# xinntao/EDVR

Hardware: AMD Instinct MI355X
Metric: EDVR-L x4 5-frame 720p clips/sec (higher is better)
Workload: dtype fp32 emulated as 2xf16 (hi+lo, 22-bit operands, 4 cross products), fp32 accumulate; 1 GPU; EDVR-L x4, 5 frames, 180x320 LR -> 720x1280, batch 10/GPU, inference; clips_per_gpu=10, global_clips=10, parallelism=clip-sharded x1, no data-path collective, world_size=1, backend=single process

## Files before the change

edvr_amd/_lib.py:

```python
import ctypes
import os

_HERE = os.path.dirname(os.path.abspath(__file__))
LIB_PATH = os.environ.get('EDVR_AMD_LIB') or os.path.join(_HERE, 'lib', 'libedvr_amd.so')

c_float_p = ctypes.c_void_p
i32, i64, f32, sz = ctypes.c_int, ctypes.c_int64, ctypes.c_float, ctypes.c_size_t
vp = ctypes.c_void_p


class ConvDesc(ctypes.Structure):
    _fields_ = [
        ('x1', vp), ('x2', vp), ('c1', i32), ('c2', i32), ('x1_img_stride', i64), ('x2_img_stride', i64),
        ('x2_div', i32), ('x2_mul', i32), ('x2_add', i32), ('n', i32), ('h', i32), ('w', i32), ('wpk', vp),
        ('bias', vp), ('co', i32), ('ks', i32), ('stride', i32), ('act', i32), ('act_from', i32), ('res1', vp),
        ('res2', vp), ('res1_img_stride', i64), ('res2_img_stride', i64), ('y', vp), ('y_img_stride', i64),
        ('out_mode', i32), ('algo', i32), ('gate', vp), ('gate_img_stride', i64), ('gate_slope', f32), ('y_scale', f32),
        ('wpk_f4', vp), ('abs_sum', vp), ('abs_sum_channels', i32), ('wpk_f4s', vp), ('x_amax', vp), ('y_amax', vp),
        ('pre', vp), ('pre_img_stride', i64), ('pre_div', i32), ('pre_mul', i32), ('pre_add', i32), ('pre_n', i32), ('wpk_ds', vp),
    ]


PROTOTYPES = {
    'edvr_version': (ctypes.c_char_p, []),
    'edvr_last_error': (ctypes.c_char_p, []),
    'edvr_check_device': (i32, []),
    'edvr_conv2d_packed_weight_elems': (sz, [i32, i32, i32]),
    'edvr_conv2d_pack_weight_f32': (i32, [vp, vp, i32, i32, i32, i32, vp]),
    'edvr_conv2d_packed_weight_f4_elems': (sz, [i32, i32]),
    'edvr_conv2d_pack_weight_f4_f32': (i32, [vp, vp, i32, i32, i32, vp]),
    'edvr_conv2d_packed_weight_f4s_elems': (sz, [i32, i32]),
    'edvr_conv2d_pack_weight_f4s_f32': (i32, [vp, vp, i32, i32, i32, vp]),
    'edvr_conv2d_packed_weight_1x1s_elems': (sz, [i32, i32]),
    'edvr_conv2d_pack_weight_1x1s_f32': (i32, [vp, vp, i32, i32, vp]),
    'edvr_conv2d_packed_weight_ds_elems': (sz, [i32, i32, i32]),
    'edvr_conv2d_pack_weight_ds_f32': (i32, [vp, vp, i32, i32, i32, vp]),
    'edvr_amax_f32': (i32, [vp, vp, i32, i64, i64, vp]),
    'edvr_pack_job_bytes': (sz, []),
    'edvr_conv2d_pack_weights_multi': (i32, [vp, i32, i32, i32, vp]),
    'edvr_conv2d_f32': (i32, [ctypes.POINTER(ConvDesc), vp]),
    'edvr_conv2d_kernel': (i32, [ctypes.POINTER(ConvDesc)]),
    'edvr_conv2d_gate_supported': (i32, [ctypes.POINTER(ConvDesc)]),
    'edvr_conv2d_abs_sum_supported': (i32, [ctypes.POINTER(ConvDesc)]),
    'edvr_conv2d_y_amax_supported': (i32, [ctypes.POINTER(ConvDesc)]),
    'edvr_conv2d_pre_supported': (i32, [ctypes.POINTER(ConvDesc)]),
    'edvr_conv2d_f4s_set_lean': (i32, [i32]),
    'edvr_conv2d_f4s_lean_items': (i32, [ctypes.POINTER(ConvDesc)]),
    'edvr_conv2d_kernel_name': (i32, [ctypes.POINTER(ConvDesc), ctypes.c_char_p, sz]),
    'edvr_conv2d_executed_flops': (i32, [ctypes.POINTER(ConvDesc), ctypes.POINTER(ctypes.c_double)]),
    'edvr_dcnv2_fwd_ws_bytes': (sz, [i32] * 12),
    'edvr_dcnv2_fwd_f32': (i32, [vp] * 6 + [i32] * 12 + [i64, i64, i32, i32, vp, sz, vp]),
    'edvr_dcnv2_fwd_split_f32': (i32, [vp] * 6 + [i32] * 12 + [i64, i64, i32, i32, vp, sz, vp, vp]),
    'edvr_dcnv2_fwd_split_applies': (i32, [vp] + [i32] * 13),
    'edvr_dcnv2_fwd_kernel_name': (i32, [vp] + [i32] * 13 + [ctypes.c_char_p, sz]),
    'edvr_dcnv2_bwd_ws_bytes': (sz, [i32] * 12),
    'edvr_dcnv2_any_ws_bytes': (sz, [i32] * 13),
    'edvr_dcnv2_fwd_any': (i32, [i32] + [vp] * 6 + [i32] * 12 + [i64, i64, vp, sz, vp]),
    'edvr_dcnv2_bwd_any': (i32, [i32] + [vp] * 10 + [i32] * 12 + [i64, i64, i64, i64, vp, sz, vp]),
    'edvr_psnr_sse_f32': (i32, [vp, vp, vp, i32, i32, i32, i32, i64, i64, i32, i32, i32, vp]),
    'edvr_ssim_partials': (sz, [i32, i32, i32]),
    'edvr_ssim_f32': (i32, [vp, vp, vp, i32, i32, i32, i32, i64, i64, i32, i32, vp]),
    'edvr_niqe_blocks': (sz, [i32, i32, i32]),
    'edvr_niqe_moments_f32': (i32, [vp, vp, i32, i32, i32, i32, i64, i32, vp]),
    'edvr_niqe_moments_u8': (i32, [vp, vp, i32, i32, i32, i64, i32, vp]),
    'edvr_frames_u8_to_f32': (i32, [vp, vp, i32, i32, i32, i32, vp, i32, vp]),
    'edvr_gather_images_f32': (i32, [vp, vp, vp, vp, i32, vp, i32, i32, vp]),
    'edvr_upsample4x_add_u8': (i32, [vp, vp, vp, i32, i32, i32, vp]),
    'edvr_f32_to_u8_hwc': (i32, [vp, vp, i32, i32, i32, i64, vp]),
    'edvr_crop_pad_frames_u8': (i32, [vp, vp, i32, i32, i32, i32, i32, i32, i32, i32, vp]),
# ... 98 lines not shown
```

edvr_amd/csrc/winograd_f4s.hip:

```cpp
#include <atomic>
#include <cstdlib>
#include <type_traits>

#include "common.h"
#include "pack.h"

#ifndef F4S_PLAIN
#define F4S_PLAIN 1
#endif

namespace edvr {

typedef float f32x16 __attribute__((ext_vector_type(16)));
typedef float f32x4 __attribute__((ext_vector_type(4)));
typedef float f32x2 __attribute__((ext_vector_type(2)));
typedef int i32x4 __attribute__((ext_vector_type(4)));
typedef _Float16 f16x8 __attribute__((ext_vector_type(8)));

__device__ __forceinline__ float max_raw_s(float a, float b) {
  float o;
  asm("v_max_f32 %0, %1, %2" : "=v"(o) : "v"(a), "v"(b));
  return o;
}

__device__ __forceinline__ void split6_f16x2(const float (&x)[6], float s, unsigned (&o)[6]) {
  asm volatile(
      "v_fma_mixlo_f16 %0, %6, %12, 0\n\tv_fma_mixlo_f16 %1, %7, %12, 0\n\tv_fma_mixlo_f16 %2, %8, %12, 0\n\t"
      "v_fma_mixlo_f16 %3, %9, %12, 0\n\tv_fma_mixlo_f16 %4, %10, %12, 0\n\tv_fma_mixlo_f16 %5, %11, %12, 0\n\t"
      "v_fma_mixhi_f16 %0, %6, %12, -%0 op_sel_hi:[0,0,1]\n\tv_fma_mixhi_f16 %1, %7, %12, -%1 op_sel_hi:[0,0,1]\n\t"
      "v_fma_mixhi_f16 %2, %8, %12, -%2 op_sel_hi:[0,0,1]\n\tv_fma_mixhi_f16 %3, %9, %12, -%3 op_sel_hi:[0,0,1]\n\t"
      "v_fma_mixhi_f16 %4, %10, %12, -%4 op_sel_hi:[0,0,1]\n\tv_fma_mixhi_f16 %5, %11, %12, -%5 op_sel_hi:[0,0,1]"
      : "=&v"(o[0]), "=&v"(o[1]), "=&v"(o[2]), "=&v"(o[3]), "=&v"(o[4]), "=&v"(o[5])
      : "v"(x[0]), "v"(x[1]), "v"(x[2]), "v"(x[3]), "v"(x[4]), "v"(x[5]), "s"(s));
}

struct WinoF4SArgs {
  edvr_conv2d_desc d;
  const unsigned *U;
  int ci, ci_real, cop, tiles_x, tiles_y, items;
  float ys, ys_gs;
  int lean;
};

#define F4S_LDS_BARRIER() asm volatile("s_waitcnt lgkmcnt(0)\n\ts_barrier" ::: "memory")

#ifdef F4S_PROF
__device__ unsigned long long f4s_prof[16 * 8];
#define F4S_NOW(v) asm volatile("s_memtime %0\n\ts_waitcnt lgkmcnt(0)" : "=s"(v)::"memory")
#define F4S_BARRIER_AT(slot)                                        \
  do {                                                              \
    unsigned long long a_, b_;                                      \
    asm volatile("s_waitcnt lgkmcnt(0)" ::: "memory");              \
    F4S_NOW(a_);                                                    \
    asm volatile("s_barrier" ::: "memory");                         \
    F4S_NOW(b_);                                                    \
    f4s_pc[slot] += (unsigned)(b_ - a_);                            \
  } while (0)
#define F4S_SPAN_BEGIN() F4S_NOW(f4s_t0)
#define F4S_SPAN_END(slot)                                          \
  do {                                                              \
    unsigned long long b_;                                          \
    F4S_NOW(b_);                                                    \
    f4s_pc[slot] += (unsigned)(b_ - f4s_t0);                        \
    f4s_t0 = b_;                                                    \
  } while (0)
#define F4S_WAIT_DMA()                                              \
  do {                                                              \
    unsigned long long a_, b_;                                      \
    F4S_NOW(a_);                                                    \
    asm volatile("s_waitcnt vmcnt(0)" ::: "memory");                \
    F4S_NOW(b_);                                                    \
    f4s_pc[4] += (unsigned)(b_ - a_);                               \
  } while (0)
#define F4S_PROF_FLUSH()                                                                                         \
  do {                                                                                                          \
    if ((threadIdx.x & 63) == 0)                                                                                \
      for (int i_ = 0; i_ < 8; ++i_) atomicAdd(&f4s_prof[(threadIdx.x >> 6) * 8 + i_], (unsigned long long)f4s_pc[i_]); \
  } while (0)
#else
#define F4S_BARRIER_AT(slot) F4S_LDS_BARRIER()
#define F4S_SPAN_BEGIN()
#define F4S_SPAN_END(slot)
#define F4S_WAIT_DMA() asm volatile("s_waitcnt vmcnt(0)" ::: "memory")
#define F4S_PROF_FLUSH()
#endif
#if defined(F4S_PROF) && F4S_PROF >= 2
#define F4S_POS_T0() unsigned long long pa_, pb_, pc_; F4S_NOW(pa_)
#define F4S_POS_T1()                                                \
  do {                                                              \
    F4S_NOW(pb_);                                                   \
    asm volatile("s_waitcnt vmcnt(5)" ::: "memory");                \
    F4S_NOW(pc_);                                                   \
    f4s_pc[5] += (unsigned)(pb_ - pa_);                             \
    f4s_pc[6] += (unsigned)(pc_ - pb_);                             \
  } while (0)
#else
#define F4S_POS_T0()
#define F4S_POS_T1()
#endif
#define F4S_BARRIER() F4S_BARRIER_AT(7)

__device__ __forceinline__ float f4s_input_scale(float amax) {
  const int be = (int)((__builtin_bit_cast(unsigned, amax) >> 23) & 255u);
  const int field = min(max(127 + 8 - (be - 127), 7), 227);
  return __builtin_bit_cast(float, (unsigned)field << 23);
}

template <int TXL>
__global__ __launch_bounds__(1024, 1) void conv3x3_winograd_f4s_kernel(const WinoF4SArgs a) {
  constexpr int TX = 1 << TXL, TY = 32 / TX;
  constexpr int BW = 4 * TX, BH = 4 * TY;
  constexpr int RROWS = BH + 2, RPIECES = TX + 2;
  static_assert(RROWS * RPIECES == 180, "a wave's region holds 2 x 180 pieces either way");
  constexpr int CK = 8;
  constexpr int VSLAB = CK * 36 * 32;
  constexpr int XSZ = 2 * 6 * 8 * 32 * 4;
  constexpr int RWAVE = 6 * 64 * 4 + 4;
  constexpr int UCHUNK = 6 * 2 * 6 * 1024;
  __shared__ __attribute__((aligned(16))) float smem[2 * VSLAB + XSZ + 4 * RWAVE + 64];
  float *const Xs = smem + 2 * VSLAB;
  float *const bias_s = smem + 2 * VSLAB + XSZ + 4 * RWAVE;

  const edvr_conv2d_desc &d = a.d;
  const int tid = threadIdx.x, lane = tid & 63, half = lane >> 5, j = lane & 31;
  const int wave = __builtin_amdgcn_readfirstlane(tid >> 6);
  const int hw = d.h * d.w, plane_bytes = hw * 4;
  const int co_blocks = (d.co + 63) / 64;
  const int n_chunks = a.ci / CK;
  constexpr int RSRC_FLAGS = 0x00020000;
  auto uniform_rsrc = [&](const void *p, int bytes) {
    const uint64_t pv = reinterpret_cast<uint64_t>(p);
    const uint64_t pu = ((uint64_t)(uint32_t)__builtin_amdgcn_readfirstlane((int)(pv >> 32)) << 32) |
                        (uint32_t)__builtin_amdgcn_readfirstlane((int)(uint32_t)pv);
    return __builtin_amdgcn_make_buffer_rsrc(reinterpret_cast<void *>(pu), (short)0, bytes, RSRC_FLAGS);
  };

  const int n_xcd = gridDim.x < 8 ? 1 : 8;
  const int xcd = n_xcd == 1 ? 0 : (int)blockIdx.x % 8, xcd_rank = n_xcd == 1 ? (int)blockIdx.x : (int)blockIdx.x / 8;
  const int xcd_wgs = n_xcd == 1 ? (int)gridDim.x : ((int)gridDim.x - xcd + 7) / 8;
  const int span = (a.items + n_xcd - 1) / n_xcd;
  const int item_end = min(a.items, (xcd + 1) * span);
  const int item_first = xcd * span + xcd_rank;
  if (item_first >= item_end) return;
#ifdef F4S_PROF
  unsigned f4s_pc[8] = {0u, 0u, 0u, 0u, 0u, 0u, 0u, 0u};
  unsigned long long f4s_t0 = 0;
#endif
  auto decode = [&](int item, int &co_blk, int &img, int &ty0, int &tx0) {
    co_blk = __builtin_amdgcn_readfirstlane((item % co_blocks) * 64);
    const int tile_blk = __builtin_amdgcn_readfirstlane((item / co_blocks) % (a.tiles_x * a.tiles_y));
    img = __builtin_amdgcn_readfirstlane(item / (co_blocks * a.tiles_x * a.tiles_y));
    ty0 = __builtin_amdgcn_readfirstlane((tile_blk / a.tiles_x) * BH);
    tx0 = __builtin_amdgcn_readfirstlane((tile_blk % a.tiles_x) * BW);
  };

  if (wave < 4) {
    __builtin_amdgcn_s_setprio(3);
    const float s_v = f4s_input_scale(__builtin_bit_cast(float, __builtin_amdgcn_readfirstlane(__builtin_bit_cast(int, *d.x_amax))));
    const float s_u_inv = __builtin_bit_cast(float, __builtin_amdgcn_readfirstlane((int)a.U[1]));
    const float unscale = s_u_inv * (1.f / s_v);
    const int p_ty = j >> TXL, p_tx = j & (TX - 1);
    typedef __attribute__((address_space(3))) void lvoid;
    constexpr int OOB = (int)0x80000000;
    float *const Rw = smem + 2 * VSLAB + XSZ + wave * RWAVE;
    int dma_off[6];
    const float *x1 = d.x1, *x2 = d.x1;
    int l_item = item_first, l_k = 0;
    auto setup = [&](int item) {
      int cb, img, ty0, tx0;
      decode(item, cb, img, ty0, tx0);
      x1 = d.x1 + (int64_t)img * d.x1_img_stride;
      x2 = x1;
      if (d.x2) {
        const int i2 = d.x2_div > 0 ? (img / d.x2_div) * d.x2_mul + d.x2_add : img;
        x2 = d.x2 + (int64_t)i2 * d.x2_img_stride;
      }
#pragma unroll
      for (int i = 0; i < 6; ++i) {
        const int q = i * 64 + lane, ch = q / 180, rem = q - ch * 180, row = rem / RPIECES, cx = rem - row * RPIECES;
        const int gy = ty0 - 1 + row, gx = tx0 - 4 + 4 * cx;
// ... 123 lines not shown
    for (int item = item_first; item < item_end; item += xcd_wgs) {
      int e_co_blk, e_img, e_ty0, e_tx0;
      decode(item, e_co_blk, e_img, e_ty0, e_tx0);
      if (d.abs_sum && e_img != asum_img) {
        asum_flush();
        asum_img = e_img;
      }
#pragma unroll 1
      for (int k = 0; k < n_chunks; ++k) {
        unsigned *Vd = Vst + (par ^ 1) * VSLAB;
        read_patch();
        advance();
        load_begin(l_k * CK);
        dma_issue();
#pragma unroll
        for (int cp = 0; cp < 3; ++cp) transform_cols(cp);
#pragma unroll
        for (int r = 0; r < 6; ++r) commit_row(Vd, r);
        F4S_BARRIER_AT(0);
        par ^= 1;
      }
      F4S_SPAN_END(2);

      const int plane = hw;
      float *y = d.y + (int64_t)e_img * d.y_img_stride;
      const float *r1 = d.res1 ? d.res1 + (int64_t)e_img * d.res1_img_stride : nullptr;
      const float *r2 = d.res2 ? d.res2 + (int64_t)e_img * d.res2_img_stride : nullptr;
      const float *gt = d.gate ? d.gate + (int64_t)e_img * d.gate_img_stride : nullptr;
      const float *pq = nullptr;
      if (d.pre) pq = d.pre + (int64_t)(d.pre_div > 0 ? (e_img / d.pre_div) * d.pre_mul + d.pre_add : e_img) * d.pre_img_stride;
      const float *rq = gt ? gt : (pq ? pq : r1);
      const float slope = d.act == EDVR_ACT_LRELU ? 0.1f : (d.act == EDVR_ACT_RELU ? 0.f : 1.f);
      const bool sig = d.act == EDVR_ACT_SIGMOID, shuffle = d.out_mode == EDVR_OUT_PIXEL_SHUFFLE2;
      const bool vec = e_tx0 + BW <= d.w;
      const int cl8 = (wave * 64 + lane) >> 5, tile = lane & 31;
      const int oy = e_ty0 + 4 * (tile >> TXL), ox = e_tx0 + 4 * (tile & (TX - 1));
      const int co_t = e_co_blk + (cl8 >> 2) * 32 + 4 * ((cl8 >> 1) & 1) + 8 * (cl8 & 1);
      const int pix = oy * d.w + ox;
      const int rows_in = d.h - oy;
      if (wave == 0) bias_s[lane] = (d.bias && e_co_blk + lane < d.co) ? d.bias[e_co_blk + lane] : 0.f;
      auto column_pass = [&](auto VEC, auto SHUF, auto PREADD) {
        constexpr bool PRE = decltype(PREADD)::value;
        constexpr bool V = decltype(VEC)::value;
        constexpr bool SHF = decltype(SHUF)::value;
        f32x4 Yprev[4];
        f32x4 rr[4];
// ... 207 lines not shown
#pragma unroll
          for (int i = 0; i < 4; ++i) __builtin_amdgcn_raw_buffer_store_b128(__builtin_bit_cast(i32x4, Y[i]), y_rs, voff[i], soff, 0);
          soff += (p & 3) == 3 ? 13 * pb : pb;
          bp += (p & 3) == 3 ? 13 : 1;
          Xb += x_step;
          x_step = -x_step;
          if (ADD && p != 7) {
#pragma unroll
            for (int i = 0; i < 4; ++i) rr[i] = __builtin_bit_cast(f32x4, __builtin_amdgcn_raw_buffer_load_b128(q_rs, voff[i], soff, 0));
          }
          if (want_amax) {
#pragma unroll
            for (int i = 0; i < 4; ++i) {
              const i32x4 yb = __builtin_bit_cast(i32x4, Y[i]);
              pmax = max(max(pmax, yb[0]), yb[1]);
              pmax = max(max(pmax, yb[2]), yb[3]);
              umax = max(max(umax, (unsigned)yb[0]), (unsigned)yb[1]);
              umax = max(max(umax, (unsigned)yb[2]), (unsigned)yb[3]);
            }
          }
        }
        amx = max(amx, max((unsigned)max(pmax, 0), umax & 0x7fffffffu));
      };
      if (lean_item) {
        auto with_add = [&](auto ACT_) {
          if (lean_f & 16) column_pass_lean(ACT_, std::integral_constant<int, 2>{});
          else if (lean_f & 8) column_pass_lean(ACT_, std::integral_constant<int, 1>{});
          else column_pass_lean(ACT_, std::integral_constant<int, 0>{});
        };
        if (lean_f & 4) with_add(std::true_type{});
        else with_add(std::false_type{});
      } else if (pq && vec) column_pass(std::true_type{}, std::false_type{}, std::true_type{});
      else if (pq) column_pass(std::false_type{}, std::false_type{}, std::true_type{});
      else if (vec && shuffle) column_pass(std::true_type{}, std::true_type{}, std::false_type{});
      else if (vec) column_pass(std::true_type{}, std::false_type{}, std::false_type{});
      else column_pass(std::false_type{}, std::false_type{}, std::false_type{});
      F4S_SPAN_END(3);
    }
    if (d.abs_sum) asum_flush();
    if (d.y_amax) {
#pragma unroll
      for (int sh = 32; sh > 0; sh >>= 1) amx = max(amx, (unsigned)__shfl_xor((int)amx, sh));
      if (lane == 0 && amx > 0u) atomicMax(reinterpret_cast<unsigned *>(d.y_amax), amx);
    }
    F4S_PROF_FLUSH();
  } else {
    const int q = wave - 4, wm = q & 1, row = q >> 1;
    const __amdgpu_buffer_rsrc_t u_rsrc = uniform_rsrc(a.U, 64 + a.cop * a.ci * 36 * 4);
    const int voff = lane * 16;
    f32x16 acc[6];
    i32x4 A[6];
    int u_base = 0, u_next = 0;
    auto item_base = [&](int co_blk) { return 64 + ((((co_blk >> 6) * n_chunks) * 6 + row) * 2 + wm) * (6 * 1024); };
    auto load_a = [&](int c, int soff) { A[c] = __builtin_bit_cast(i32x4, __builtin_amdgcn_raw_buffer_load_b128(u_rsrc, voff, soff + c * 1024, 0)); };
    int co_blk, img_, ty_, tx_;
    decode(item_first, co_blk, img_, ty_, tx_);
    u_base = item_base(co_blk);
#pragma unroll
    for (int c = 0; c < 6; ++c) load_a(c, u_base);
#pragma unroll
    for (int c = 0; c < 6; ++c)
#pragma unroll
      for (int r = 0; r < 16; ++r) acc[c][r] = 0.f;
    F4S_BARRIER();

    int par = 0;
    const unsigned *const Vst = reinterpret_cast<const unsigned *>(smem);
    unsigned v_addr = (unsigned)(size_t)(__attribute__((address_space(3))) const unsigned *)(Vst + 4 * half * 36 * 32 + row * 6 * 32 + j);
    int v_step = __builtin_amdgcn_readfirstlane(VSLAB * 4);
    F4S_SPAN_BEGIN();
    for (int item = item_first; item < item_end; item += xcd_wgs) {
      {
        const int nx = item + xcd_wgs;
        decode(nx < item_end ? nx : item, co_blk, img_, ty_, tx_);
        u_next = item_base(co_blk);
      }
#pragma unroll 1
      for (int k = 0; k < n_chunks; ++k) {
        const int soff_nxt = k + 1 < n_chunks ? u_base + (k + 1) * UCHUNK : u_next;
#pragma unroll
        for (int c = 0; c < 6; ++c) {
          int b0, b1, b2, b3;
          F4S_POS_T0();
          asm volatile("ds_read_b32 %0, %4 offset:%5\n\tds_read_b32 %1, %4 offset:%6\n\tds_read_b32 %2, %4 offset:%7\n\tds_read_b32 %3, %4 offset:%8\n\t"
                       "s_waitcnt lgkmcnt(0)"
                       : "=&v"(b0), "=&v"(b1), "=&v"(b2), "=&v"(b3)
                       : "v"(v_addr), "n"(c * 128), "n"(36 * 128 + c * 128), "n"(2 * 36 * 128 + c * 128), "n"(3 * 36 * 128 + c * 128)
                       : "memory");
          F4S_POS_T1();
          const f16x8 B = __builtin_bit_cast(f16x8, i32x4{b0, b1, b2, b3});
          acc[c] = __builtin_amdgcn_mfma_f32_32x32x16_f16(__builtin_bit_cast(f16x8, A[c]), B, acc[c], 0, 0, 0);
          asm volatile("v_alignbit_b32 %0, %0, %0, 16\n\tv_alignbit_b32 %1, %1, %1, 16\n\tv_alignbit_b32 %2, %2, %2, 16\n\tv_alignbit_b32 %3, %3, %3, 16"
                       : "+v"(A[c][0]), "+v"(A[c][1]), "+v"(A[c][2]), "+v"(A[c][3]));
          acc[c] = __builtin_amdgcn_mfma_f32_32x32x16_f16(__builtin_bit_cast(f16x8, A[c]), B, acc[c], 0, 0, 0);
          __builtin_amdgcn_sched_barrier(0);
          load_a(c, soff_nxt);
          __builtin_amdgcn_sched_barrier(0);
        }
        v_addr += v_step;
        v_step = -v_step;
        F4S_BARRIER_AT(0);
        par ^= 1;
      }
      u_base = u_next;
      F4S_SPAN_END(2);
      int lane_e = lane;
      asm volatile("" : "+v"(lane_e));
      float *const Xw = Xs + ((row * 8 + wm * 4 + (lane_e >> 5) * 2) * 32 + (lane_e & 31)) * 4;
#pragma unroll
      for (int p = 0; p < 8; ++p) {
        float *Xb = Xw + (p & 1) * (XSZ / 2);
#pragma unroll
        for (int rr = 0; rr < 2; ++rr) {
          const int r = (p & 3) + 4 * (2 * (p >> 2) + rr);
          const float m0 = acc[0][r], m1 = acc[1][r], m2 = acc[2][r], m3 = acc[3][r], m4 = acc[4][r], m5 = acc[5][r];
          const float s1 = m1 + m2, d1 = m1 - m2, s2 = m3 + m4, d2 = m3 - m4;
          f32x4 T;
          T[0] = m0 + s1 + s2;
          T[1] = __builtin_fmaf(2.f, d2, d1);
          T[2] = __builtin_fmaf(4.f, s2, s1);
          T[3] = __builtin_fmaf(8.f, d2, d1) + m5;
          *reinterpret_cast<f32x4 *>(Xb + rr * 32 * 4) = T;
        }
        F4S_BARRIER_AT(1);
      }
#pragma unroll
      for (int c = 0; c < 6; ++c) load_a(c, u_base);
#pragma unroll
      for (int c = 0; c < 6; ++c)
#pragma unroll
        for (int r = 0; r < 16; ++r) acc[c][r] = 0.f;
      F4S_SPAN_END(3);
    }
    F4S_PROF_FLUSH();
  }
}

__global__ __launch_bounds__(1024) void winograd_f4s_weight_scale_kernel(const float *__restrict__ w, unsigned *__restrict__ U, int64_t total) {
  __shared__ float red[16];
  float m = 0.f;
  for (int64_t i = threadIdx.x; i < total; i += 1024) m = fmaxf(m, fabsf(w[i]));
#pragma unroll
  for (int sh = 32; sh > 0; sh >>= 1) m = fmaxf(m, __shfl_xor(m, sh));
  if ((threadIdx.x & 63) == 0) red[threadIdx.x >> 6] = m;
  __syncthreads();
  if (threadIdx.x == 0) {
    for (int i = 1; i < 16; ++i) m = fmaxf(m, red[i]);
    const unsigned field = f4s_weight_scale_field(__builtin_bit_cast(unsigned, m));
    U[0] = field << 23;
    U[1] = (254u - field) << 23;
    for (int i = 2; i < 16; ++i) U[i] = 0u;
  }
}

__global__ void winograd_f4s_weight_kernel(const float *__restrict__ w, unsigned *__restrict__ U, int co, int ci, int cop, int cip, int transpose_flip) {
// ... 60 lines not shown
bool winograd_f4s_eligible(const edvr_conv2d_desc &d) {
  if (!winograd_f4s_supported(d)) return false;
  if (d.algo == EDVR_CONV_WINOGRAD_F4S) return true;
  if (d.algo != EDVR_CONV_AUTO || !winograd_f4s_enabled()) return false;
  return d.co >= 48 && d.c1 + d.c2 >= 32 && d.w >= 32 && d.h >= 8;
}

static int f4s_geometry(const edvr_conv2d_desc &d, int &tiles_x, int &tiles_y, bool &tx8) {
  const int64_t pad16 = (int64_t)cdiv(d.w, 64) * 64 * cdiv(d.h, 8) * 8, pad8 = (int64_t)cdiv(d.w, 32) * 32 * cdiv(d.h, 16) * 16;
  tx8 = pad8 < pad16;
  tiles_x = cdiv(d.w, tx8 ? 32 : 64);
  tiles_y = cdiv(d.h, tx8 ? 16 : 8);
  return tiles_x * tiles_y * cdiv(d.co, 64) * d.n;
}

static std::atomic<int> &f4s_lean_switch() {
  static std::atomic<int> on([]() {
    const char *e = getenv("EDVR_F4S_LEAN");
    return (e && e[0] == '0') ? 0 : 1;
  }());
  return on;
}

static int f4s_lean_launch(const edvr_conv2d_desc &d) {
  if (!f4s_lean_switch().load(std::memory_order_relaxed)) return 0;
  if (d.out_mode != EDVR_OUT_NCHW || d.gate || d.abs_sum || d.res2) return 0;
  if (d.act != EDVR_ACT_NONE && d.act != EDVR_ACT_RELU && d.act != EDVR_ACT_LRELU) return 0;
  if ((int64_t)d.h * d.w * 4 * 64 >= ((int64_t)1 << 31)) return 0;
  return 1 | (d.y_amax ? 2 : 0) | (d.act != EDVR_ACT_NONE ? 4 : 0) | (d.pre ? 16 : (d.res1 ? 8 : 0));
}

static bool f4s_lean_item(const edvr_conv2d_desc &d, int co_blk, int ty0, int tx0, int bw, int bh) {
  return tx0 + bw <= d.w && ty0 + bh <= d.h && co_blk + 64 <= d.co && (d.act == EDVR_ACT_NONE || d.act_from <= co_blk);
}

int winograd_f4s_lean_items(const edvr_conv2d_desc &d) {
  if (!f4s_lean_launch(d)) return 0;
  int tiles_x, tiles_y;
  bool tx8;
  f4s_geometry(d, tiles_x, tiles_y, tx8);
  const int bw = tx8 ? 32 : 64, bh = tx8 ? 16 : 8;
  int per_img = 0;
  for (int cb = 0; cb < d.co; cb += 64)
    for (int ty = 0; ty < tiles_y; ++ty)
      for (int tx = 0; tx < tiles_x; ++tx) per_img += f4s_lean_item(d, cb, ty * bh, tx * bw, bw, bh) ? 1 : 0;
  return per_img * d.n;
}

double winograd_f4s_executed_flops(const edvr_conv2d_desc &d) {
  int tx, ty;
  bool tx8;
  const double items = f4s_geometry(d, tx, ty, tx8);
  return items * ((d.c1 + d.c2 + 7) / 8) * 144.0 * 32768.0;
}

int winograd_f4s_launch(const edvr_conv2d_desc &d, hipStream_t stream) {
  WinoF4SArgs a;
  a.d = d;
  a.U = reinterpret_cast<const unsigned *>(d.wpk_f4s);
  a.ci_real = d.c1 + d.c2;
  a.ci = (a.ci_real + 7) / 8 * 8;
  a.cop = (d.co + 63) / 64 * 64;
  a.ys = d.y_scale == 0.f ? 1.f : d.y_scale;
  a.ys_gs = a.ys * d.gate_slope;
  bool tx8;
  a.items = f4s_geometry(d, a.tiles_x, a.tiles_y, tx8);
  a.lean = f4s_lean_launch(d);
  static const int n_cu = []() {
    int dev = 0, n = 256;
    hipDeviceProp_t prop;
    if (hipGetDevice(&dev) == hipSuccess && hipGetDeviceProperties(&prop, dev) == hipSuccess) n = prop.multiProcessorCount;
    return n;
  }();
  const dim3 grid(std::min(a.items, n_cu));
  if (tx8) hipLaunchKernelGGL(conv3x3_winograd_f4s_kernel<3>, grid, dim3(1024), 0, stream, a);
  else hipLaunchKernelGGL(conv3x3_winograd_f4s_kernel<4>, grid, dim3(1024), 0, stream, a);
  return check_launch("conv3x3_winograd_f4s_kernel");
}

}

extern "C" {

#ifdef F4S_PROF
int edvr_f4s_prof_read(unsigned long long *host, int reset) {
  int rc = (int)hipMemcpyFromSymbol(host, HIP_SYMBOL(edvr::f4s_prof), sizeof(unsigned long long) * 128);
  if (rc == 0 && reset) {
    static unsigned long long zero[128];
    rc = (int)hipMemcpyToSymbol(HIP_SYMBOL(edvr::f4s_prof), zero, sizeof(zero));
  }
  return rc;
}
#endif

int edvr_conv2d_f4s_set_lean(int on) { return edvr::f4s_lean_switch().exchange(on ? 1 : 0); }

int edvr_conv2d_f4s_lean_items(const edvr_conv2d_desc *d) {
  return (d && edvr::conv2d_select(*d) == edvr::CONV_F4S) ? edvr::winograd_f4s_lean_items(*d) : 0;
}

size_t edvr_conv2d_packed_weight_f4s_elems(int co, int ci) { return 16 + (size_t)((co + 63) / 64 * 64) * ((ci + 7) / 8 * 8) * 36; }

int edvr_conv2d_pack_weight_f4s_f32(const float *w, void *wpk_f4s, int co, int ci, int transpose_flip, edvr_stream_t stream) {
  EDVR_REQUIRE(w && wpk_f4s && co > 0 && ci > 0, "pack_weight_f4s: bad arguments");
  const int cop = (co + 63) / 64 * 64, cip = (ci + 7) / 8 * 8;
  const int64_t total = (int64_t)cip * cop;
  unsigned *U = reinterpret_cast<unsigned *>(wpk_f4s);
  hipLaunchKernelGGL(edvr::winograd_f4s_weight_scale_kernel, dim3(1), dim3(1024), 0, edvr::as_stream(stream), w, U, (int64_t)co * ci * 9);
  hipLaunchKernelGGL(edvr::winograd_f4s_weight_kernel, dim3((unsigned)std::min<int64_t>(edvr::cdiv64(total, 256), 4096)), dim3(256), 0,
                     edvr::as_stream(stream), w, U, co, ci, cop, cip, transpose_flip);
  return edvr::check_launch("winograd_f4s_weight_kernel");
}

int edvr_amax_f32(const float *x, float *amax, int n, int64_t per_img, int64_t img_stride, edvr_stream_t stream) {
  EDVR_REQUIRE(x && amax && n > 0 && per_img > 0, "amax: bad arguments");
  if (img_stride == per_img || n == 1) {
    per_img *= n;
    n = 1;
// ... 10 lines not shown
```

include/edvr_amd.h:

```cpp
#ifndef EDVR_AMD_H
#define EDVR_AMD_H

#include <stddef.h>
#include <stdint.h>

#ifdef __cplusplus
extern "C" {
#endif

#define EDVR_OK 0
#define EDVR_ERR_ARG (-1)
#define EDVR_ERR_UNSUPPORTED (-2)
#define EDVR_ERR_LAUNCH (-3)
#define EDVR_ERR_WORKSPACE (-4)

typedef void *edvr_stream_t;

const char *edvr_version(void);
const char *edvr_last_error(void);
int edvr_check_device(void);

#define EDVR_ACT_NONE 0
#define EDVR_ACT_RELU 1
#define EDVR_ACT_LRELU 2
// ... 60 lines not shown
int edvr_conv2d_pack_weight_f4s_f32(const float *w, void *wpk_f4s, int co, int ci, int transpose_flip, edvr_stream_t stream);
size_t edvr_conv2d_packed_weight_1x1s_elems(int co, int ci);
int edvr_conv2d_pack_weight_1x1s_f32(const float *w, void *wpk_1x1s, int co, int ci, edvr_stream_t stream);
size_t edvr_conv2d_packed_weight_ds_elems(int co, int ci, int ks);
int edvr_conv2d_pack_weight_ds_f32(const float *w, void *wpk_ds, int co, int ci, int ks, edvr_stream_t stream);
int edvr_amax_f32(const float *x, float *amax, int n, int64_t per_img, int64_t img_stride, edvr_stream_t stream);
size_t edvr_pack_job_bytes(void);
int edvr_conv2d_pack_weights_multi(const void *jobs, int n_jobs, int total_blocks, int split_parity, edvr_stream_t stream);
int edvr_conv2d_f32(const edvr_conv2d_desc *d, edvr_stream_t stream);
#define EDVR_CONV_KERNEL_SMALL 0
#define EDVR_CONV_KERNEL_F4S 1
#define EDVR_CONV_KERNEL_F4 2
#define EDVR_CONV_KERNEL_F2 3
#define EDVR_CONV_KERNEL_1X1_SPLIT 4
#define EDVR_CONV_KERNEL_1X1_STREAM 5
#define EDVR_CONV_KERNEL_DIRECT_SPLIT 6
#define EDVR_CONV_KERNEL_DIRECT 7
int edvr_conv2d_kernel(const edvr_conv2d_desc *d);
int edvr_conv2d_gate_supported(const edvr_conv2d_desc *d);
int edvr_conv2d_y_amax_supported(const edvr_conv2d_desc *d);
int edvr_conv2d_abs_sum_supported(const edvr_conv2d_desc *d);
int edvr_conv2d_pre_supported(const edvr_conv2d_desc *d);
int edvr_conv2d_f4s_set_lean(int on);
int edvr_conv2d_f4s_lean_items(const edvr_conv2d_desc *d);
int edvr_conv2d_kernel_name(const edvr_conv2d_desc *d, char *buf, size_t buf_len);
int edvr_conv2d_executed_flops(const edvr_conv2d_desc *d, double *flops);

#define EDVR_HW(h, w) ((int)(h) | (((int)(w) + 1) << 16))

size_t edvr_dcnv2_fwd_ws_bytes(int B, int C, int H, int W, int Co, int kh, int kw, int stride, int pad, int dil,
                               int groups, int dg);
int edvr_dcnv2_fwd_f32(const float *x, const float *offset, const float *mask, const float *weight,
                       const float *bias, float *y, int B, int C, int H, int W, int Co, int kh, int kw, int stride,
                       int pad, int dil, int groups, int dg, int64_t offset_bstride, int64_t mask_bstride, int act,
                       int halo_hint, void *ws, size_t ws_bytes, edvr_stream_t stream);

int edvr_dcnv2_fwd_split_f32(const float *x, const float *offset, const float *mask, const float *weight, const float *bias,
                             float *y, int B, int C, int H, int W, int Co, int kh, int kw, int stride, int pad, int dil, int groups,
                             int dg, int64_t offset_bstride, int64_t mask_bstride, int act, int halo_hint, void *ws, size_t ws_bytes,
                             const float *xm_amax, edvr_stream_t stream);
int edvr_dcnv2_fwd_split_applies(const float *x, int B, int C, int H, int W, int Co, int kh, int kw, int stride, int pad, int dil, int groups,
                                 int dg, int halo_hint);
int edvr_dcnv2_fwd_kernel_name(const float *x, int B, int C, int H, int W, int Co, int kh, int kw, int stride, int pad, int dil,
                               int groups, int dg, int halo_hint, char *buf, size_t buf_len);

size_t edvr_dcnv2_bwd_ws_bytes(int B, int C, int H, int W, int Co, int kh, int kw, int stride, int pad, int dil,
// ... 188 lines not shown
```

Baseline: 105.5 clips/s.

## Let MFMA waves share the Winograd output transform and hand-schedule the multiply loop

```diff
diff --git a/edvr_amd/_lib.py b/edvr_amd/_lib.py
--- a/edvr_amd/_lib.py
+++ b/edvr_amd/_lib.py
@@ -45,6 +45,7 @@
     'edvr_conv2d_y_amax_supported': (i32, [ctypes.POINTER(ConvDesc)]),
     'edvr_conv2d_pre_supported': (i32, [ctypes.POINTER(ConvDesc)]),
     'edvr_conv2d_f4s_set_lean': (i32, [i32]),
+    'edvr_conv2d_f4s_set_allwaves': (i32, [i32]),
     'edvr_conv2d_f4s_lean_items': (i32, [ctypes.POINTER(ConvDesc)]),
     'edvr_conv2d_kernel_name': (i32, [ctypes.POINTER(ConvDesc), ctypes.c_char_p, sz]),
     'edvr_conv2d_executed_flops': (i32, [ctypes.POINTER(ConvDesc), ctypes.POINTER(ctypes.c_double)]),
diff --git a/edvr_amd/csrc/winograd_f4s.hip b/edvr_amd/csrc/winograd_f4s.hip
--- a/edvr_amd/csrc/winograd_f4s.hip
+++ b/edvr_amd/csrc/winograd_f4s.hip
@@ -40,6 +40,7 @@
   int ci, ci_real, cop, tiles_x, tiles_y, items;
   float ys, ys_gs;
   int lean;
+  int allwaves;
 };
 
 #define F4S_LDS_BARRIER() asm volatile("s_waitcnt lgkmcnt(0)\n\ts_barrier" ::: "memory")
@@ -84,20 +85,6 @@
 #define F4S_WAIT_DMA() asm volatile("s_waitcnt vmcnt(0)" ::: "memory")
 #define F4S_PROF_FLUSH()
 #endif
-#if defined(F4S_PROF) && F4S_PROF >= 2
-#define F4S_POS_T0() unsigned long long pa_, pb_, pc_; F4S_NOW(pa_)
-#define F4S_POS_T1()                                                \
-  do {                                                              \
-    F4S_NOW(pb_);                                                   \
-    asm volatile("s_waitcnt vmcnt(5)" ::: "memory");                \
-    F4S_NOW(pc_);                                                   \
-    f4s_pc[5] += (unsigned)(pb_ - pa_);                             \
-    f4s_pc[6] += (unsigned)(pc_ - pb_);                             \
-  } while (0)
-#else
-#define F4S_POS_T0()
-#define F4S_POS_T1()
-#endif
 #define F4S_BARRIER() F4S_BARRIER_AT(7)
 
 __device__ __forceinline__ float f4s_input_scale(float amax) {
@@ -117,13 +104,24 @@
   constexpr int XSZ = 2 * 6 * 8 * 32 * 4;
   constexpr int RWAVE = 6 * 64 * 4 + 4;
   constexpr int UCHUNK = 6 * 2 * 6 * 1024;
-  __shared__ __attribute__((aligned(16))) float smem[2 * VSLAB + XSZ + 4 * RWAVE + 64];
+  __shared__ __attribute__((aligned(16))) float smem[2 * VSLAB + XSZ + 4 * RWAVE + 64 + 1024];
   float *const Xs = smem + 2 * VSLAB;
   float *const bias_s = smem + 2 * VSLAB + XSZ + 4 * RWAVE;
+  unsigned *const amx_s = reinterpret_cast<unsigned *>(bias_s + 64);
 
   const edvr_conv2d_desc &d = a.d;
-  const int tid = threadIdx.x, lane = tid & 63, half = lane >> 5, j = lane & 31;
-  const int wave = __builtin_amdgcn_readfirstlane(tid >> 6);
+  typedef const WinoF4SArgs __attribute__((address_space(4))) *KArgs;
+  auto kargs_here = []() {
+    KArgs kp = (KArgs)__builtin_amdgcn_kernarg_segment_ptr();
+    asm volatile("" : "+s"(kp));
+    return kp;
+  };
+  const int wave = __builtin_amdgcn_readfirstlane((int)threadIdx.x >> 6);
+  auto lane_here = []() {
+    int l;
+    asm volatile("v_mbcnt_lo_u32_b32 %0, -1, 0\n\tv_mbcnt_hi_u32_b32 %0, -1, %0" : "=v"(l));
+    return l;
+  };
   const int hw = d.h * d.w, plane_bytes = hw * 4;
   const int co_blocks = (d.co + 63) / 64;
   const int n_chunks = a.ci / CK;
@@ -154,8 +152,83 @@
     tx0 = __builtin_amdgcn_readfirstlane((tile_blk % a.tiles_x) * BW);
   };
 
+  auto item_allwaves = [&](int co_blk, int ty0, int tx0) {
+    return a.allwaves && (a.lean & 1) && tx0 + BW <= d.w && ty0 + BH <= d.h && co_blk + 64 <= d.co && (!(a.lean & 4) || d.act_from <= co_blk);
+  };
+  struct Share {
+    __amdgpu_buffer_rsrc_t y_rs, q_rs;
+    const float *Xb, *bp;
+    int voff, soff, pb, w4, flags;
+    float us, sl, ys;
+    int pmax;
+    unsigned umax;
+    float rr[4];
+  };
+  auto share_load = [&](Share &st, int so) {
+#pragma unroll
+    for (int i = 0; i < 4; ++i) st.rr[i] = __builtin_bit_cast(float, __builtin_amdgcn_raw_buffer_load_b32(st.q_rs, st.voff, so + i * st.w4, 0));
+  };
+  auto share_setup = [&](Share &st, float *y_img, const float *q_img, int lean_f, int pb, int w4, int co_blk, int ty0, int tx0, int lane, float unscale, float slope) {
+    const int t = (wave & 1) * 64 + lane, tile = t >> 2, col = t & 3, cl8 = wave >> 1;
+    const int cw = (cl8 >> 2) * 32 + 4 * ((cl8 >> 1) & 1) + 8 * (cl8 & 1);
+    const int64_t blk = (int64_t)co_blk * (pb >> 2);
+    st.y_rs = uniform_rsrc(y_img + blk, 64 * pb);
+    st.q_rs = uniform_rsrc(q_img ? q_img + blk : y_img, q_img ? 64 * pb : 0);
+    st.voff = (ty0 + 4 * (tile >> TXL)) * w4 + (tx0 + 4 * (tile & (TX - 1)) + col) * 4;
+    st.soff = cw * pb;
+    st.pb = pb;
+    st.w4 = w4;
+    st.flags = lean_f;
+    st.Xb = Xs + wave * 64 + lane;
+    st.bp = bias_s + cw;
+    st.us = unscale;
+    st.sl = slope;
+    st.ys = a.ys;
+    st.pmax = 0;
+    st.umax = 0u;
+    if (lean_f & 24) share_load(st, st.soff);
+  };
+  auto share_phase = [&](Share &st, int p) {
+    const float *Xp = st.Xb + (p & 1) * (XSZ / 2);
+    const float t0 = Xp[0], t1 = Xp[1024], t2 = Xp[2 * 1024], t3 = Xp[3 * 1024], t4 = Xp[4 * 1024], t5 = Xp[5 * 1024];
+    const int pc = (p & 3) + 16 * (p >> 2);
+    const float b = st.bp[pc];
+    const float s1 = t1 + t2, d1 = t1 - t2, s2 = t3 + t4, d2 = t3 - t4;
+    float y[4];
+    y[0] = __builtin_fmaf(t0 + s1 + s2, st.us, b);
+    y[1] = __builtin_fmaf(__builtin_fmaf(2.f, d2, d1), st.us, b);
+    y[2] = __builtin_fmaf(__builtin_fmaf(4.f, s2, s1), st.us, b);
+    y[3] = __builtin_fmaf(__builtin_fmaf(8.f, d2, d1) + t5, st.us, b);
+    if (st.flags & 16) {
+#pragma unroll
+      for (int i = 0; i < 4; ++i) y[i] += st.rr[i];
+    }
+    if (st.flags & 4) {
+#pragma unroll
+      for (int i = 0; i < 4; ++i) y[i] = max_raw_s(y[i], y[i] * st.sl);
+    }
+    if (st.flags & 8) {
+#pragma unroll
+      for (int i = 0; i < 4; ++i) y[i] = __builtin_fmaf(y[i], st.ys, st.rr[i]);
+    }
+    const int so = st.soff + pc * st.pb;
+#pragma unroll
+    for (int i = 0; i < 4; ++i) __builtin_amdgcn_raw_buffer_store_b32(__builtin_bit_cast(int, y[i]), st.y_rs, st.voff, so + i * st.w4, 0);
+    if ((st.flags & 24) && p != 7) share_load(st, st.soff + ((p + 1 & 3) + 16 * (p + 1 >> 2)) * st.pb);
+    if (st.flags & 2) {
+#pragma unroll
+      for (int i = 0; i < 4; ++i) {
+        const int yb = __builtin_bit_cast(int, y[i]);
+        st.pmax = max(st.pmax, yb);
+        st.umax = max(st.umax, (unsigned)yb);
+      }
+    }
+  };
+  auto share_amax = [&](const Share &st) { return max((unsigned)max(st.pmax, 0), st.umax & 0x7fffffffu); };
+
   if (wave < 4) {
     __builtin_amdgcn_s_setprio(3);
+    const int lane = (int)threadIdx.x & 63, half = lane >> 5, j = lane & 31;
     const float s_v = f4s_input_scale(__builtin_bit_cast(float, __builtin_amdgcn_readfirstlane(__builtin_bit_cast(int, *d.x_amax))));
     const float s_u_inv = __builtin_bit_cast(float, __builtin_amdgcn_readfirstlane((int)a.U[1]));
     const float unscale = s_u_inv * (1.f / s_v);
@@ -325,6 +398,9 @@
       }
       F4S_SPAN_END(2);
 
+      const KArgs kp = kargs_here();
+      const auto &a = *kp;
+      const auto &d = kp->d;
       const int plane = hw;
       float *y = d.y + (int64_t)e_img * d.y_img_stride;
       const float *r1 = d.res1 ? d.res1 + (int64_t)e_img * d.res1_img_stride : nullptr;
@@ -578,7 +654,16 @@
         }
         amx = max(amx, max((unsigned)max(pmax, 0), umax & 0x7fffffffu));
       };
-      if (lean_item) {
+      if (lean_item && a.allwaves) {
+        Share st;
+        share_setup(st, y, (lean_f & 16) ? pq : ((lean_f & 8) ? r1 : nullptr), lean_f, pb, w4, e_co_blk, e_ty0, e_tx0, lane, unscale, slope);
+#pragma unroll 1
+        for (int p = 0; p < 8; ++p) {
+          F4S_BARRIER_AT(1);
+          share_phase(st, p);
+        }
+        amx = max(amx, share_amax(st));
+      } else if (lean_item) {
         auto with_add = [&](auto ACT_) {
           if (lean_f & 16) column_pass_lean(ACT_, std::integral_constant<int, 2>{});
           else if (lean_f & 8) column_pass_lean(ACT_, std::integral_constant<int, 1>{});
@@ -603,24 +688,27 @@
   } else {
     const int q = wave - 4, wm = q & 1, row = q >> 1;
     const __amdgpu_buffer_rsrc_t u_rsrc = uniform_rsrc(a.U, 64 + a.cop * a.ci * 36 * 4);
-    const int voff = lane * 16;
+    const int lane = lane_here(), half = lane >> 5, j = lane & 31;
+    amx_s[wave * 64 + lane] = 0u;
+    int voff = lane * 16;
     f32x16 acc[6];
     i32x4 A[6];
     int u_base = 0, u_next = 0;
     auto item_base = [&](int co_blk) { return 64 + ((((co_blk >> 6) * n_chunks) * 6 + row) * 2 + wm) * (6 * 1024); };
-    auto load_a = [&](int c, int soff) { A[c] = __builtin_bit_cast(i32x4, __builtin_amdgcn_raw_buffer_load_b128(u_rsrc, voff, soff + c * 1024, 0)); };
     int co_blk, img_, ty_, tx_;
     decode(item_first, co_blk, img_, ty_, tx_);
     u_base = item_base(co_blk);
-#pragma unroll
-    for (int c = 0; c < 6; ++c) load_a(c, u_base);
-#pragma unroll
-    for (int c = 0; c < 6; ++c)
-#pragma unroll
-      for (int r = 0; r < 16; ++r) acc[c][r] = 0.f;
+    auto zero_acc = [&]() {
+      float z = 0.f;
+      asm volatile("" : "+v"(z));
+#pragma unroll
+      for (int c = 0; c < 6; ++c)
+#pragma unroll
+        for (int r = 0; r < 16; ++r) acc[c][r] = z;
+    };
+    zero_acc();
     F4S_BARRIER();
 
-    int par = 0;
     const unsigned *const Vst = reinterpret_cast<const unsigned *>(smem);
     unsigned v_addr = (unsigned)(size_t)(__attribute__((address_space(3))) const unsigned *)(Vst + 4 * half * 36 * 32 + row * 6 * 32 + j);
     int v_step = __builtin_amdgcn_readfirstlane(VSLAB * 4);
@@ -631,62 +719,111 @@
         decode(nx < item_end ? nx : item, co_blk, img_, ty_, tx_);
         u_next = item_base(co_blk);
       }
-#pragma unroll 1
-      for (int k = 0; k < n_chunks; ++k) {
-        const int soff_nxt = k + 1 < n_chunks ? u_base + (k + 1) * UCHUNK : u_next;
-#pragma unroll
-        for (int c = 0; c < 6; ++c) {
-          int b0, b1, b2, b3;
-          F4S_POS_T0();
-          asm volatile("ds_read_b32 %0, %4 offset:%5\n\tds_read_b32 %1, %4 offset:%6\n\tds_read_b32 %2, %4 offset:%7\n\tds_read_b32 %3, %4 offset:%8\n\t"
-                       "s_waitcnt lgkmcnt(0)"
-                       : "=&v"(b0), "=&v"(b1), "=&v"(b2), "=&v"(b3)
-                       : "v"(v_addr), "n"(c * 128), "n"(36 * 128 + c * 128), "n"(2 * 36 * 128 + c * 128), "n"(3 * 36 * 128 + c * 128)
-                       : "memory");
-          F4S_POS_T1();
-          const f16x8 B = __builtin_bit_cast(f16x8, i32x4{b0, b1, b2, b3});
-          acc[c] = __builtin_amdgcn_mfma_f32_32x32x16_f16(__builtin_bit_cast(f16x8, A[c]), B, acc[c], 0, 0, 0);
-          asm volatile("v_alignbit_b32 %0, %0, %0, 16\n\tv_alignbit_b32 %1, %1, %1, 16\n\tv_alignbit_b32 %2, %2, %2, 16\n\tv_alignbit_b32 %3, %3, %3, 16"
-                       : "+v"(A[c][0]), "+v"(A[c][1]), "+v"(A[c][2]), "+v"(A[c][3]));
-          acc[c] = __builtin_amdgcn_mfma_f32_32x32x16_f16(__builtin_bit_cast(f16x8, A[c]), B, acc[c], 0, 0, 0);
-          __builtin_amdgcn_sched_barrier(0);
-          load_a(c, soff_nxt);
-          __builtin_amdgcn_sched_barrier(0);
-        }
-        v_addr += v_step;
-        v_step = -v_step;
-        F4S_BARRIER_AT(0);
-        par ^= 1;
+      {
+        voff = lane_here() * 16;
+        int cnt = n_chunks - 1, soff = u_base + UCHUNK, soff_hi;
+#define F4S_MUL_POS(ACC, A0, A1, A2, A3, O0, O1, O2, O3, VM, TAIL)                                                                       \
+  "ds_read_b32 v122, %[va] offset:" #O0 "\n\tds_read_b32 v123, %[va] offset:" #O1 "\n\tds_read_b32 v124, %[va] offset:" #O2             \
+  "\n\tds_read_b32 v125, %[va] offset:" #O3 "\n\ts_waitcnt lgkmcnt(0)\n\ts_waitcnt vmcnt(" #VM ")\n\t"                                \
+  "v_mfma_f32_32x32x16_f16 %[" #ACC "], v[" #A0 ":" #A3 "], v[122:125], %[" #ACC "]\n\t"                                                 \
+  "v_alignbit_b32 v" #A0 ", v" #A0 ", v" #A0 ", 16\n\tv_alignbit_b32 v" #A1 ", v" #A1 ", v" #A1 ", 16\n\t"                              \
+  "v_alignbit_b32 v" #A2 ", v" #A2 ", v" #A2 ", 16\n\tv_alignbit_b32 v" #A3 ", v" #A3 ", v" #A3 ", 16\n\ts_nop 1\n\t"                 \
+  "v_mfma_f32_32x32x16_f16 %[" #ACC "], v[" #A0 ":" #A3 "], v[122:125], %[" #ACC "]\n\t" TAIL
+#define F4S_MUL_LOAD(A0, A3, SO, OFF) "buffer_load_dwordx4 v[" #A0 ":" #A3 "], %[vo], %[rs], %[" #SO "] offen offset:" #OFF "\n\t"
+#define F4S_MUL_STEP "v_add_u32 %[va], %[vs], %[va]\n\ts_sub_u32 %[vs], 0, %[vs]\n\ts_barrier\n\t"
+        asm volatile(
+            "s_sub_u32 %[sh], %[so], 0x12000\n\t"
+            F4S_MUL_LOAD(98, 101, sh, 0) F4S_MUL_LOAD(102, 105, sh, 1024) F4S_MUL_LOAD(106, 109, sh, 2048) F4S_MUL_LOAD(110, 113, sh, 3072)
+            "s_add_u32 %[sh], %[sh], 0x1000\n\t"
+            F4S_MUL_LOAD(114, 117, sh, 0) F4S_MUL_LOAD(118, 121, sh, 1024)
+            "s_cmp_eq_u32 %[cnt], 0\n\t"
+            "s_cbranch_scc1 .Lf4s_last_%=\n"
+            ".Lf4s_loop_%=:\n\t"
+            "s_add_u32 %[sh], %[so], 0x1000\n\t"
+            F4S_MUL_POS(c0, 98, 99, 100, 101, 0, 4608, 9216, 13824, 5, F4S_MUL_LOAD(98, 101, so, 0))
+            F4S_MUL_POS(c1, 102, 103, 104, 105, 128, 4736, 9344, 13952, 5, F4S_MUL_LOAD(102, 105, so, 1024))
+            F4S_MUL_POS(c2, 106, 107, 108, 109, 256, 4864, 9472, 14080, 5, F4S_MUL_LOAD(106, 109, so, 2048))
+            F4S_MUL_POS(c3, 110, 111, 112, 113, 384, 4992, 9600, 14208, 5, F4S_MUL_LOAD(110, 113, so, 3072))
+            F4S_MUL_POS(c4, 114, 115, 116, 117, 512, 5120, 9728, 14336, 5, F4S_MUL_LOAD(114, 117, sh, 0))
+            F4S_MUL_POS(c5, 118, 119, 120, 121, 640, 5248, 9856, 14464, 5, F4S_MUL_LOAD(118, 121, sh, 1024))
+            F4S_MUL_STEP
+            "s_add_u32 %[so], %[so], 0x12000\n\t"
+            "s_sub_u32 %[cnt], %[cnt], 1\n\t"
+            "s_cmp_lg_u32 %[cnt], 0\n\t"
+            "s_cbranch_scc1 .Lf4s_loop_%=\n"
+            ".Lf4s_last_%=:\n\t"
+            F4S_MUL_POS(c0, 98, 99, 100, 101, 0, 4608, 9216, 13824, 5, "")
+            F4S_MUL_POS(c1, 102, 103, 104, 105, 128, 4736, 9344, 13952, 4, "")
+            F4S_MUL_POS(c2, 106, 107, 108, 109, 256, 4864, 9472, 14080, 3, "")
+            F4S_MUL_POS(c3, 110, 111, 112, 113, 384, 4992, 9600, 14208, 2, "")
+            F4S_MUL_POS(c4, 114, 115, 116, 117, 512, 5120, 9728, 14336, 1, "")
+            F4S_MUL_POS(c5, 118, 119, 120, 121, 640, 5248, 9856, 14464, 0, "")
+            F4S_MUL_STEP
+            "s_nop 15\n\t"
+            : [c0] "+v"(acc[0]), [c1] "+v"(acc[1]), [c2] "+v"(acc[2]), [c3] "+v"(acc[3]), [c4] "+v"(acc[4]), [c5] "+v"(acc[5]),
+              "=&{v[98:101]}"(A[0]), "=&{v[102:105]}"(A[1]), "=&{v[106:109]}"(A[2]), "=&{v[110:113]}"(A[3]), "=&{v[114:117]}"(A[4]),
+              "=&{v[118:121]}"(A[5]), [va] "+v"(v_addr), [vs] "+s"(v_step), [cnt] "+s"(cnt), [so] "+s"(soff), [sh] "=&s"(soff_hi)
+            : [vo] "v"(voff), [rs] "s"(u_rsrc)
+            : "memory", "scc", "v122", "v123", "v124", "v125");
+#undef F4S_MUL_POS
+#undef F4S_MUL_LOAD
+#undef F4S_MUL_STEP
+        static_assert(UCHUNK == 0x12000 && 36 * 32 * 4 == 4608, "the asm text holds the chunk size and the B offsets as literals");
       }
       u_base = u_next;
       F4S_SPAN_END(2);
-      int lane_e = lane;
-      asm volatile("" : "+v"(lane_e));
+      const int lane_e = lane_here();
       float *const Xw = Xs + ((row * 8 + wm * 4 + (lane_e >> 5) * 2) * 32 + (lane_e & 31)) * 4;
-#pragma unroll
-      for (int p = 0; p < 8; ++p) {
-        float *Xb = Xw + (p & 1) * (XSZ / 2);
-#pragma unroll
-        for (int rr = 0; rr < 2; ++rr) {
-          const int r = (p & 3) + 4 * (2 * (p >> 2) + rr);
-          const float m0 = acc[0][r], m1 = acc[1][r], m2 = acc[2][r], m3 = acc[3][r], m4 = acc[4][r], m5 = acc[5][r];
-          const float s1 = m1 + m2, d1 = m1 - m2, s2 = m3 + m4, d2 = m3 - m4;
-          f32x4 T;
-          T[0] = m0 + s1 + s2;
-          T[1] = __builtin_fmaf(2.f, d2, d1);
-          T[2] = __builtin_fmaf(4.f, s2, s1);
-          T[3] = __builtin_fmaf(8.f, d2, d1) + m5;
-          *reinterpret_cast<f32x4 *>(Xb + rr * 32 * 4) = T;
+      const KArgs kp = kargs_here();
+      const auto &a = *kp;
+      const auto &d = kp->d;
+      int c_cb, c_img, c_ty0, c_tx0;
+      decode(item, c_cb, c_img, c_ty0, c_tx0);
+      auto row_pass = [&](auto AW_) {
+        constexpr bool AW = decltype(AW_)::value;
+        Share st;
+        if (AW) {
+          const float s_v = f4s_input_scale(__builtin_bit_cast(float, __builtin_amdgcn_readfirstlane(__builtin_bit_cast(int, *d.x_amax))));
+          const float s_u_inv = __builtin_bit_cast(float, __builtin_amdgcn_readfirstlane((int)a.U[1]));
+          int lean_f = a.lean, pb = plane_bytes, w4 = d.w * 4;
+          asm volatile("" : "+s"(lean_f), "+s"(pb), "+s"(w4));
+          const float *q = nullptr;
+          if (lean_f & 16) q = d.pre + (int64_t)(d.pre_div > 0 ? (c_img / d.pre_div) * d.pre_mul + d.pre_add : c_img) * d.pre_img_stride;
+          else if (lean_f & 8) q = d.res1 + (int64_t)c_img * d.res1_img_stride;
+          share_setup(st, d.y + (int64_t)c_img * d.y_img_stride, q, lean_f, pb, w4, c_cb, c_ty0, c_tx0, lane_e, s_u_inv * (1.f / s_v),
+                      d.act == EDVR_ACT_LRELU ? 0.1f : (d.act == EDVR_ACT_RELU ? 0.f : 1.f));
         }
-        F4S_BARRIER_AT(1);
-      }
-#pragma unroll
-      for (int c = 0; c < 6; ++c) load_a(c, u_base);
-#pragma unroll
-      for (int c = 0; c < 6; ++c)
-#pragma unroll
-        for (int r = 0; r < 16; ++r) acc[c][r] = 0.f;
+#pragma unroll
+        for (int p = 0; p < 8; ++p) {
+          float *Xb = Xw + (p & 1) * (XSZ / 2);
+#pragma unroll
+          for (int rr = 0; rr < 2; ++rr) {
+            const int r = (p & 3) + 4 * (2 * (p >> 2) + rr);
+            const float m0 = acc[0][r], m1 = acc[1][r], m2 = acc[2][r], m3 = acc[3][r], m4 = acc[4][r], m5 = acc[5][r];
+            const float s1 = m1 + m2, d1 = m1 - m2, s2 = m3 + m4, d2 = m3 - m4;
+            f32x4 T;
+            T[0] = m0 + s1 + s2;
+            T[1] = __builtin_fmaf(2.f, d2, d1);
+            T[2] = __builtin_fmaf(4.f, s2, s1);
+            T[3] = __builtin_fmaf(8.f, d2, d1) + m5;
+            *reinterpret_cast<f32x4 *>(Xb + rr * 32 * 4) = T;
+          }
+          F4S_BARRIER_AT(1);
+          __builtin_amdgcn_sched_barrier(0);
+          if (AW) share_phase(st, p);
+        }
+        if (AW && (st.flags & 2)) __hip_atomic_fetch_max(amx_s + wave * 64 + lane_e, share_amax(st), __ATOMIC_RELAXED, __HIP_MEMORY_SCOPE_WORKGROUP);
+      };
+      if (item_allwaves(c_cb, c_ty0, c_tx0)) row_pass(std::true_type{});
+      else row_pass(std::false_type{});
+      zero_acc();
       F4S_SPAN_END(3);
+    }
+    if (d.y_amax && a.allwaves) {
+      unsigned amx = amx_s[wave * 64 + lane_here()];
+#pragma unroll
+      for (int sh = 32; sh > 0; sh >>= 1) amx = max(amx, (unsigned)__shfl_xor((int)amx, sh));
+      if (lane_here() == 0 && amx > 0u) atomicMax(reinterpret_cast<unsigned *>(d.y_amax), amx);
     }
     F4S_PROF_FLUSH();
   }
@@ -793,6 +930,14 @@
   return on;
 }
 
+static std::atomic<int> &f4s_allwaves_switch() {
+  static std::atomic<int> on([]() {
+    const char *e = getenv("EDVR_F4S_ALLWAVES");
+    return (e && e[0] != '0' && e[0] != 0) ? 1 : 0;
+  }());
+  return on;
+}
+
 static int f4s_lean_launch(const edvr_conv2d_desc &d) {
   if (!f4s_lean_switch().load(std::memory_order_relaxed)) return 0;
   if (d.out_mode != EDVR_OUT_NCHW || d.gate || d.abs_sum || d.res2) return 0;
@@ -837,6 +982,7 @@
   bool tx8;
   a.items = f4s_geometry(d, a.tiles_x, a.tiles_y, tx8);
   a.lean = f4s_lean_launch(d);
+  a.allwaves = a.lean ? f4s_allwaves_switch().load(std::memory_order_relaxed) : 0;
   static const int n_cu = []() {
     int dev = 0, n = 256;
     hipDeviceProp_t prop;
@@ -865,6 +1011,8 @@
 #endif
 
 int edvr_conv2d_f4s_set_lean(int on) { return edvr::f4s_lean_switch().exchange(on ? 1 : 0); }
+
+int edvr_conv2d_f4s_set_allwaves(int on) { return edvr::f4s_allwaves_switch().exchange(on ? 1 : 0); }
 
 int edvr_conv2d_f4s_lean_items(const edvr_conv2d_desc *d) {
   return (d && edvr::conv2d_select(*d) == edvr::CONV_F4S) ? edvr::winograd_f4s_lean_items(*d) : 0;
diff --git a/include/edvr_amd.h b/include/edvr_amd.h
--- a/include/edvr_amd.h
+++ b/include/edvr_amd.h
@@ -106,6 +106,7 @@
 int edvr_conv2d_abs_sum_supported(const edvr_conv2d_desc *d);
 int edvr_conv2d_pre_supported(const edvr_conv2d_desc *d);
 int edvr_conv2d_f4s_set_lean(int on);
+int edvr_conv2d_f4s_set_allwaves(int on);
 int edvr_conv2d_f4s_lean_items(const edvr_conv2d_desc *d);
 int edvr_conv2d_kernel_name(const edvr_conv2d_desc *d, char *buf, size_t buf_len);
 int edvr_conv2d_executed_flops(const edvr_conv2d_desc *d, double *flops);
```

New measurement: 105.0 clips/s. No clear change (-0.4%).
